# jhbastek/PhysicsInformedDiffusionModels

Hardware: NVIDIA H100
Metric: train samples/s Darcy 64x64 PIDM (higher is better)
Workload: dtype bf16

## Files before the change

include/pidm.h:

```cpp
#ifndef PIDM_H_
#define PIDM_H_

#ifdef __cplusplus
extern "C" {
#endif

#ifndef PIDM_F32
#define PIDM_F32 0
#define PIDM_BF16 1
#endif

const char* pidm_last_error(void);
int pidm_version(void);

int pidm_qsample(const float* x0, const float* noise, const long long* t, const float* sqrt_ab,
                 const float* sqrt_1mab, float* xt, int B, int per_sample, void* stream);
int pidm_posterior_step(const float* x_t, const float* x0_pred, const float* z, float* out, float coef1, float coef2,
                        float sigma, long long n, void* stream);
int pidm_axpby_per_sample(const float* a, const float* x, const float* b, const float* y, const float* c,
                          const float* z, float* out, int B, int per_sample, void* stream);
int pidm_ddim_coefs(const long long* t, const long long* t_next, const float* posterior_mean_coef1,
                    const float* posterior_mean_coef2, const float* sqrt_recip_alphas, const float* noise_mean_coeff,
                    const float* alphas_prod, float* coef_x0, float* coef_x, int B, void* stream);
int pidm_scale(const float* x, const float* alpha_dev, float* out, long long n, void* stream);
// ... 34 lines not shown
                     int transposed, int dtype, void* stream);
int pidm_conv2d_wgrad_simt(const void* x, const void* dy, float* dw, float* dbias, int B, int H, int W, int Cin,
                           int Cin_real, int Ho, int Wo, int Cout, int KH, int KW, int stride, int pad, int transposed,
                           long long w_stride_n, long long w_stride_c, int dtype, void* stream);
int pidm_debug_set_trace(void* buf);
int pidm_conv2d_tc_general(const void* x, const void* w_packed, const float* bias, const void* residual, void* y, int B,
                           int H, int W, int Cin, int Ho, int Wo, int Cout, int KH, int KW, int stride, int pad,
                           int transposed, float* gn_sums, int gn_groups, int gn_sums_zeroed, void* stream);
int pidm_conv2d_tc_general_supported(int B, int H, int W, int Cin, int Ho, int Wo, int Cout, int KH, int KW, int stride,
                                     int pad, int transposed);
int pidm_conv2d_wgrad_tc(const void* a, const void* b, float* dw, int B, int HA, int WA, int CA, int CA_real, int GH,
                         int GW, int CB, int KH, int KW, int a_stride, int pad, long long s_row, long long s_col,
                         void* stream);
int pidm_conv2d_wgrad_tc_supported(int B, int GH, int GW, int CA, int CB, int KH, int KW, int a_stride);
int pidm_colsum(const void* x, float* out, long long M, int C, int dtype, void* stream);

int pidm_groupnorm_silu_fwd(const void* x, const float* gamma, const float* beta, const float* scale_shift,
                            const void* residual, void* y, float* sums, int stats_precomputed, int B, int HW, int C, int G,
                            float eps, int dtype, void* stream);
int pidm_groupnorm_silu_bwd(const void* x, const void* dy, const float* sums, const float* gamma, const float* beta,
                            const float* scale_shift, void* dx, float* dgamma, float* dbeta, float* d_scale_shift,
                            float* dbias_of_producer, float* workspace, int B, int HW, int C, int G, float eps,
                            int dtype, void* stream);
int pidm_layernorm_c_fwd(const void* x, const float* gamma, void* y, long long M, int C, float eps, int dtype, void* stream);
int pidm_layernorm_c_bwd(const void* x, const void* dy, const float* gamma, void* dx, float* dgamma,
                         const void* dx_residual , long long M, int C,
                         float eps, int dtype, void* stream);

int pidm_linattn_fused_supported(int C, int heads, int N, int dtype);
int pidm_linattn_fused_workspace_floats(int B, int N);
int pidm_linattn_fused_fwd(const void* xn, const void* w_qkv, void* out, float* ctx, float* kmax, float* kzinv,
                           float* workspace, int B, int N, void* stream);
int pidm_linattn_fused_bwd(const void* xn, const void* w_qkv, const void* dout, const float* ctx, const float* kmax,
                           const float* kzinv, void* dqkv, float* dctx, int B, int N, void* stream);
int pidm_linattn_workspace_floats(int B, int N, int heads);
int pidm_linattn_fwd(const void* qkv, void* out, float* ctx, float* kmax, float* kzinv, float* workspace, int B, int N,
                     int heads, int dtype, void* stream);
int pidm_linattn_bwd(const void* qkv, const void* dout, const float* ctx, const float* kmax, const float* kzinv,
                     void* dqkv, float* dctx_scratch, int B, int N, int heads, int dtype, void* stream);
int pidm_attn_fwd(const void* qkv, void* out, int B, int n_tokens, int heads, int dtype, void* stream);
int pidm_attn_bwd(const void* qkv, const void* dout, void* dqkv, int B, int n_tokens, int heads, int dtype, void* stream);

int pidm_time_embed_fwd(const long long* t, const float* W1, const float* b1, const float* W2, const float* b2,
                        float* emb, float* h1, float* temb, float* silu_t, int B, int dim, int td, void* stream);
int pidm_time_embed_bwd(const float* d_silu_t, const float* emb, const float* h1, const float* temb, const float* W2,
                        float* dW1, float* db1, float* dW2, float* db2, float* workspace, int B, int dim, int td,
                        int parts, void* stream);
int pidm_mlp_entry_size(void);
int pidm_block_mlps_fwd(const void* table_dev, int n_entries, int max_rows, const float* silu_t, int B, int td,
                        void* stream);
int pidm_block_mlps_bwd(const void* table_dev, int n_entries, int max_rows, const float* silu_t, float* d_silu_t, int B,
                        int td, int parts, void* stream);

int pidm_head_fwd(const void* x, const float* w, const float* bias, float* y, int B, int HW, int C, int O,
                  int sigmoid_last, int dtype, void* stream);
int pidm_head_bwd(const void* x, const float* w, const float* y, const float* dy, void* dx, float* dw, float* db, int B,
                  int HW, int C, int O, int sigmoid_last, int dtype, void* stream);

int pidm_sumsq(const float* x, long long n, float* out, float* workspace, void* stream);
int pidm_adam_ema_step(float* param, float* grad, float* exp_avg, float* exp_avg_sq, float* ema_shadow, long long n,
                       float lr, double beta1, double beta2, float eps, int step, int* step_counter_dev,
                       const float* grad_norm_sq_dev, float grad_scale, float max_norm, float ema_mu,
                       int ema_first_step, int zero_grad, void* stream);

int pidm_mechanics_residual_fwd(const float* u, const float* rho, const float* bcs, const float* KE, float* residual,
                                float* compliance, int B, int nel, void* stream);
int pidm_mechanics_residual_bwd(const float* u, const float* rho, const float* bcs, const float* KE,
// ... 15 lines not shown
```

physicsinformeddiffusionmodels_b200/_lib.py:

```python
import ctypes
import os

import torch

_HERE = os.path.dirname(os.path.abspath(__file__))
LIB_PATH = os.path.join(_HERE, 'libpidm.so')

P = ctypes.c_void_p
I = ctypes.c_int
L = ctypes.c_longlong
F = ctypes.c_float
D = ctypes.c_double

_SIGS = {
    'pidm_qsample': [P, P, P, P, P, P, I, I, P],
    'pidm_posterior_step': [P, P, P, P, F, F, F, L, P],
    'pidm_scale': [P, P, P, L, P],
    'pidm_ddim_coefs': [P, P, P, P, P, P, P, P, P, I, P],
    'pidm_axpby_per_sample': [P, P, P, P, P, P, P, I, I, P],
    'pidm_toy_pidm_loss': [P, P, P, P, P, P, P, P, F, F, F, F, P, P, P, P, P, I, I, P],
    'pidm_fd_stencil': [P, P, I, I, I, F, F, P],
    'pidm_darcy_residual_fwd': [P, P, P, I, I, F, I, I, P],
    'pidm_darcy_residual_bwd': [P, P, P, P, I, I, F, I, I, P],
    'pidm_darcy_jacobian_max': [P, P, I, I, F, I, I, P],
    'pidm_darcy_pidm_loss': [P, P, P, P, P, P, P, F, F, P, P, P, I, I, F, I, I, P],
    'pidm_nchw_to_nhwc': [P, P, I, I, I, I, I, P],
    'pidm_nhwc_to_nchw': [P, P, I, I, I, I, I, P],
    'pidm_add': [P, P, P, L, I, P],
    'pidm_gelu_fwd': [P, P, L, I, P],
    'pidm_gelu_bwd': [P, P, P, L, I, P],
    'pidm_concat_channels': [P, P, P, L, I, I, I, P],
    'pidm_split_channels': [P, P, P, L, I, I, I, P],
    'pidm_pack_entry_size': [],
    'pidm_pack_weights': [P, I, I, P],
    'pidm_pack_pair_entry_size': [],
    'pidm_pack_weights_pairs': [P, P, I, I, I, I, P],
    'pidm_conv2d_simt': [P, P, P, P, P, I, I, I, I, I, I, I, I, I, I, I, I, I, P],
    'pidm_conv2d_wgrad_simt': [P, P, P, P, I, I, I, I, I, I, I, I, I, I, I, I, I, L, L, I, P],
    'pidm_debug_set_trace': [P],
    'pidm_conv2d_tc_general': [P, P, P, P, P, I, I, I, I, I, I, I, I, I, I, I, I, P, I, I, P],
    'pidm_conv2d_tc_general_supported': [I, I, I, I, I, I, I, I, I, I, I, I],
    'pidm_conv2d_wgrad_tc': [P, P, P, I, I, I, I, I, I, I, I, I, I, I, I, L, L, P],
    'pidm_conv2d_wgrad_tc_supported': [I, I, I, I, I, I, I, I],
    'pidm_colsum': [P, P, L, I, I, P],
    'pidm_groupnorm_silu_fwd': [P, P, P, P, P, P, P, I, I, I, I, I, F, I, P],
    'pidm_groupnorm_silu_bwd': [P, P, P, P, P, P, P, P, P, P, P, P, I, I, I, I, F, I, P],
    'pidm_layernorm_c_fwd': [P, P, P, L, I, F, I, P],
    'pidm_layernorm_c_bwd': [P, P, P, P, P, P, L, I, F, I, P],
    'pidm_linattn_workspace_floats': [I, I, I],
    'pidm_linattn_fused_supported': [I, I, I, I],
    'pidm_linattn_fused_workspace_floats': [I, I],
    'pidm_linattn_fused_fwd': [P, P, P, P, P, P, P, I, I, P],
    'pidm_linattn_fused_bwd': [P, P, P, P, P, P, P, P, I, I, P],
    'pidm_linattn_fwd': [P, P, P, P, P, P, I, I, I, I, P],
    'pidm_linattn_bwd': [P, P, P, P, P, P, P, I, I, I, I, P],
    'pidm_attn_fwd': [P, P, I, I, I, I, P],
    'pidm_attn_bwd': [P, P, P, I, I, I, I, P],
    'pidm_time_embed_fwd': [P, P, P, P, P, P, P, P, P, I, I, I, P],
    'pidm_time_embed_bwd': [P, P, P, P, P, P, P, P, P, P, I, I, I, I, P],
    'pidm_mlp_entry_size': [],
    'pidm_block_mlps_fwd': [P, I, I, P, I, I, P],
    'pidm_block_mlps_bwd': [P, I, I, P, P, I, I, I, P],
    'pidm_head_fwd': [P, P, P, P, I, I, I, I, I, I, P],
    'pidm_head_bwd': [P, P, P, P, P, P, P, I, I, I, I, I, I, P],
    'pidm_sumsq': [P, L, P, P, P],
    'pidm_adam_ema_step': [P, P, P, P, P, L, F, D, D, F, I, P, P, F, F, F, I, I, P],
    'pidm_mechanics_residual_fwd': [P, P, P, P, P, P, I, I, P],
    'pidm_mechanics_residual_bwd': [P, P, P, P, P, P, P, P, P, I, I, P],
    'pidm_mech_pidm_loss': [P, P, P, P, P, P, P, P, P, F, F, F, F, P, P, P, P, P, I, I, P],
    'pidm_bilinear_resize_fwd': [P, P, I, I, I, P],
    'pidm_bilinear_resize_bwd': [P, P, I, I, I, P],
    'pidm_version': [],
}
_VALUE_RETURN = {'pidm_pack_entry_size', 'pidm_pack_pair_entry_size', 'pidm_mlp_entry_size', 'pidm_linattn_workspace_floats', 'pidm_version',
                 'pidm_linattn_fused_supported', 'pidm_linattn_fused_workspace_floats',
                 'pidm_conv2d_tc_supported', 'pidm_conv2d_wgrad_tc_supported', 'pidm_conv2d_tc_general_supported'}

if not os.path.exists(LIB_PATH):
    raise ImportError(f'{LIB_PATH} is missing: build it with `python __graft_entry__.py` (nvcc, sm_90a). '
                      'There is no CPU / PyTorch fallback for the PIDM hot path.')

_lib = ctypes.CDLL(LIB_PATH)
_lib.pidm_last_error.restype = ctypes.c_char_p
_lib.pidm_last_error.argtypes = []
for _n, _a in _SIGS.items():
    _f = getattr(_lib, _n)
# ... 39 lines not shown
```

physicsinformeddiffusionmodels_b200/csrc/attention_fused.cu:

```cuda
#define PIDM_PDL_GROUP 1
#include "common.cuh"
#include "mma_util.cuh"
#include "pidm.h"

namespace pidm {

constexpr int LF_C = 32;

__device__ __forceinline__ uint32_t movm_t(uint32_t x) {
    uint32_t y;
    asm volatile("movmatrix.sync.aligned.m8n8.trans.b16 %0, %1;" : "=r"(y) : "r"(x));
    return y;
}

__device__ __forceinline__ void load_w_frags(uint32_t (&w)[2][4][2], const __nv_bfloat16* __restrict__ Wrows, int lane) {
    const int g = lane >> 2, t = lane & 3;
#pragma unroll
    for (int ks = 0; ks < 2; ++ks)
#pragma unroll
        for (int nt = 0; nt < 4; ++nt) {
            const uint32_t* row = reinterpret_cast<const uint32_t*>(Wrows + (size_t)(nt * 8 + g) * LF_C + ks * 16 + 2 * t);
            w[ks][nt][0] = __ldg(row);
            w[ks][nt][1] = __ldg(row + 4);
        }
// ... 300 lines not shown
        __syncwarp();
        issue(it + LFO_STAGES);
        float cq[2][4][4];
        project<2>(cq, ax, wq);
#pragma unroll
        for (int mt = 0; mt < 2; ++mt) {
            frag_softmax(cq[mt], scale);
            uint32_t a[2][4];
            c_to_a(a, cq[mt]);
            float c[4][4];
#pragma unroll
            for (int i = 0; i < 4; ++i)
#pragma unroll
                for (int k = 0; k < 4; ++k) c[i][k] = 0.f;
#pragma unroll
            for (int ks = 0; ks < 2; ++ks)
#pragma unroll
                for (int nt = 0; nt < 4; ++nt) mma_bf16(c[nt], a[ks], bf[ks][nt][0], bf[ks][nt][1]);
#pragma unroll
            for (int nt = 0; nt < 4; ++nt) {
                __nv_bfloat16* o = Os + (size_t)(mt * 16 + g) * LW_PITCH + nt * 8 + 2 * t;
                *reinterpret_cast<uint32_t*>(o) = pack_bf16(c[nt][0], c[nt][1]);
                *reinterpret_cast<uint32_t*>(o + 8 * LW_PITCH) = pack_bf16(c[nt][2], c[nt][3]);
            }
        }
        __syncwarp();
        lw_store<32>(odst + (size_t)it * 32 * LM_HID, LM_HID, Os, lane);
        __syncwarp();
    }
}

constexpr int LFB_ROWS = 16;
constexpr int LFB_STAGES = 4;
constexpr int LFB_STAGE_ELEMS = 2 * LFB_ROWS * LW_PITCH;
constexpr int LFB_OUT_ELEMS = 3 * LFB_ROWS * LW_PITCH;
__global__ void __launch_bounds__(256) laf_bwd_kernel(const __nv_bfloat16* __restrict__ xn, const __nv_bfloat16* __restrict__ W,
                                                      const __nv_bfloat16* __restrict__ dout, const float* __restrict__ ctx,
                                                      const float* __restrict__ dctx, const float* __restrict__ kmax,
                                                      const float* __restrict__ kzinv, __nv_bfloat16* __restrict__ dqkv,
                                                      int N, int chunk_px, float scale) {
    pdl_trigger();
    pdl_wait();
    extern __shared__ __align__(16) unsigned char raw[];
    const int b = blockIdx.y, chunk = blockIdx.x, lane = threadIdx.x & 31, h = threadIdx.x >> 5;
    __nv_bfloat16* ring = reinterpret_cast<__nv_bfloat16*>(raw) + (size_t)h * (LFB_STAGES * LFB_STAGE_ELEMS + LFB_OUT_ELEMS);
    __nv_bfloat16* Os = ring + LFB_STAGES * LFB_STAGE_ELEMS;
    float* scd = reinterpret_cast<float*>(raw + (size_t)LM_HEADS * (LFB_STAGES * LFB_STAGE_ELEMS + LFB_OUT_ELEMS) * 2) + h * LM_D;
    const int n_begin = chunk * chunk_px, n_end = min(N, n_begin + chunk_px);
    const int n_tiles = (n_end - n_begin) / LFB_ROWS;
    const size_t pix0 = (size_t)b * N + n_begin;
    const __nv_bfloat16* xsrc = xn + pix0 * LF_C;
    const __nv_bfloat16* gsrc = dout + pix0 * LM_HID + h * LM_D;
    __nv_bfloat16* ddst = dqkv + pix0 * 3 * LM_HID + h * LM_D;
    auto issue = [&](int it) {
        if (it < n_tiles) {
            __nv_bfloat16* buf = ring + (size_t)(it % LFB_STAGES) * LFB_STAGE_ELEMS;
            lw_issue<LFB_ROWS>(buf, xsrc + (size_t)it * LFB_ROWS * LF_C, LF_C, lane);
            lw_issue<LFB_ROWS>(buf + LFB_ROWS * LW_PITCH, gsrc + (size_t)it * LFB_ROWS * LM_HID, LM_HID, lane);
        }
        cp_commit();
    };
#pragma unroll
    for (int s = 0; s < LFB_STAGES; ++s) issue(s);
    const float* cg = ctx + ((size_t)b * LM_HEADS + h) * LM_D * LM_D;
    const float* dg = dctx + ((size_t)b * LM_HEADS + h) * LM_D * LM_D;
    {
        float s = 0.f;
#pragma unroll
        for (int e = 0; e < LM_D; e += 4) {
            const float4 x = *reinterpret_cast<const float4*>(dg + lane * LM_D + e);
            const float4 y = *reinterpret_cast<const float4*>(cg + lane * LM_D + e);
            s += x.x * y.x + x.y * y.y + x.z * y.z + x.w * y.w;
        }
        scd[lane] = s;
    }
    __syncwarp();
    float Mc[8], Zc[8], cdc[8];
    load_cols(Mc, kmax + (size_t)b * LM_HID + h * LM_D, lane);
    load_cols(Zc, kzinv + (size_t)b * LM_HID + h * LM_D, lane);
    load_cols(cdc, scd, lane);
    uint32_t wq[2][4][2], wk[2][4][2], wv[2][4][2];
    load_w_frags(wq, W + (size_t)(h * LM_D) * LF_C, lane);
    load_w_frags(wk, W + (size_t)(LM_HID + h * LM_D) * LF_C, lane);
    load_w_frags(wv, W + (size_t)(2 * LM_HID + h * LM_D) * LF_C, lane);
    uint32_t bc[2][4][2], bd[2][4][2], bt[2][4][2];
#pragma unroll
    for (int ks = 0; ks < 2; ++ks)
#pragma unroll
        for (int nt = 0; nt < 4; ++nt) {
            frag_b_global<false>(bc[ks][nt], cg, ks * 16, nt * 8, lane);
            frag_b_global<false>(bd[ks][nt], dg, ks * 16, nt * 8, lane);
            frag_b_global<true>(bt[ks][nt], dg, ks * 16, nt * 8, lane);
        }
    const int g = lane >> 2, t = lane & 3;
    const float invN = 1.f / (float)N;
    __nv_bfloat16* Oq = Os;
    __nv_bfloat16* Ok = Os + LFB_ROWS * LW_PITCH;
    __nv_bfloat16* Ov = Os + 2 * LFB_ROWS * LW_PITCH;
    for (int it = 0; it < n_tiles; ++it) {
        cp_wait<LFB_STAGES - 1>();
        __syncwarp();
        const __nv_bfloat16* buf = ring + (size_t)(it % LFB_STAGES) * LFB_STAGE_ELEMS;
        uint32_t ax[1][2][4], ag[2][4];
        load_x_frags<1>(ax, buf, lane);
        frag_a_rowmajor(ag[0], buf + LFB_ROWS * LW_PITCH, LW_PITCH, 0, 0, lane);
        frag_a_rowmajor(ag[1], buf + LFB_ROWS * LW_PITCH, LW_PITCH, 0, 16, lane);
        __syncwarp();
        issue(it + LFB_STAGES);
        float c1[1][4][4], c2[4][4];
        project<1>(c1, ax, wq);
        frag_softmax(c1[0], 1.f);
#pragma unroll
        for (int nt = 0; nt < 4; ++nt) {
#pragma unroll
            for (int i = 0; i < 4; ++i) c2[nt][i] = 0.f;
#pragma unroll
            for (int ks = 0; ks < 2; ++ks) mma_bf16(c2[nt], ag[ks], bc[ks][nt][0], bc[ks][nt][1]);
        }
#pragma unroll
        for (int half = 0; half < 2; ++half) {
            float dot = 0.f;
#pragma unroll
            for (int nt = 0; nt < 4; ++nt)
                dot += c1[0][nt][half * 2] * c2[nt][half * 2] + c1[0][nt][half * 2 + 1] * c2[nt][half * 2 + 1];
            dot += __shfl_xor_sync(0xffffffffu, dot, 1);
            dot += __shfl_xor_sync(0xffffffffu, dot, 2);
#pragma unroll
            for (int nt = 0; nt < 4; ++nt)
                *reinterpret_cast<uint32_t*>(Oq + (g + half * 8) * LW_PITCH + nt * 8 + 2 * t) =
                    pack_bf16(scale * c1[0][nt][half * 2] * (c2[nt][half * 2] - dot),
                              scale * c1[0][nt][half * 2 + 1] * (c2[nt][half * 2 + 1] - dot));
        }
        uint32_t av[2][4], ak[2][4];
        project<1>(c1, ax, wv);
        c_to_a(av, c1[0]);
#pragma unroll
        for (int nt = 0; nt < 4; ++nt) {
#pragma unroll
            for (int i = 0; i < 4; ++i) c2[nt][i] = 0.f;
#pragma unroll
            for (int ks = 0; ks < 2; ++ks) mma_bf16(c2[nt], av[ks], bd[ks][nt][0], bd[ks][nt][1]);
        }
        project<1>(c1, ax, wk);
#pragma unroll
        for (int nt = 0; nt < 4; ++nt)
#pragma unroll
            for (int i = 0; i < 4; ++i)
                c1[0][nt][i] = __expf(c1[0][nt][i] - Mc[nt * 2 + (i & 1)]) * Zc[nt * 2 + (i & 1)];
        c_to_a(ak, c1[0]);
#pragma unroll
        for (int half = 0; half < 2; ++half)
#pragma unroll
            for (int nt = 0; nt < 4; ++nt)
                *reinterpret_cast<uint32_t*>(Ok + (g + half * 8) * LW_PITCH + nt * 8 + 2 * t) =
                    pack_bf16(c1[0][nt][half * 2] * (c2[nt][half * 2] * invN - cdc[nt * 2]),
                              c1[0][nt][half * 2 + 1] * (c2[nt][half * 2 + 1] * invN - cdc[nt * 2 + 1]));
#pragma unroll
        for (int nt = 0; nt < 4; ++nt) {
#pragma unroll
            for (int i = 0; i < 4; ++i) c2[nt][i] = 0.f;
#pragma unroll
            for (int ks = 0; ks < 2; ++ks) mma_bf16(c2[nt], ak[ks], bt[ks][nt][0], bt[ks][nt][1]);
        }
#pragma unroll
        for (int half = 0; half < 2; ++half)
#pragma unroll
            for (int nt = 0; nt < 4; ++nt)
                *reinterpret_cast<uint32_t*>(Ov + (g + half * 8) * LW_PITCH + nt * 8 + 2 * t) =
                    pack_bf16(c2[nt][half * 2] * invN, c2[nt][half * 2 + 1] * invN);
        __syncwarp();
        __nv_bfloat16* d = ddst + (size_t)it * LFB_ROWS * 3 * LM_HID;
        lw_store<LFB_ROWS>(d, 3 * LM_HID, Oq, lane);
        lw_store<LFB_ROWS>(d + LM_HID, 3 * LM_HID, Ok, lane);
        lw_store<LFB_ROWS>(d + 2 * LM_HID, 3 * LM_HID, Ov, lane);
        __syncwarp();
    }
}

constexpr size_t LAF_STATS_SMEM = (size_t)LM_HEADS * LFS_STAGES * LW_TILE * 2;
constexpr size_t LAF_OUT_SMEM = (size_t)LM_HEADS * (LFO_STAGES + 1) * LW_TILE * 2;
constexpr size_t LAF_BWD_SMEM = (size_t)LM_HEADS * (LFB_STAGES * LFB_STAGE_ELEMS + LFB_OUT_ELEMS) * 2 + (size_t)LM_HEADS * LM_D * 4;

static int laf_attrs() {
    static bool done = false;
    if (!done) {
        PIDM_CUDA(cudaFuncSetAttribute(laf_kmax_kernel, cudaFuncAttributeMaxDynamicSharedMemorySize, (int)LAF_STATS_SMEM));
        PIDM_CUDA(cudaFuncSetAttribute(laf_ctx_kernel<0>, cudaFuncAttributeMaxDynamicSharedMemorySize, (int)LfcCfg<0>::SMEM));
        PIDM_CUDA(cudaFuncSetAttribute(laf_ctx_kernel<1>, cudaFuncAttributeMaxDynamicSharedMemorySize, (int)LfcCfg<1>::SMEM));
        PIDM_CUDA(cudaFuncSetAttribute(laf_out_kernel, cudaFuncAttributeMaxDynamicSharedMemorySize, (int)LAF_OUT_SMEM));
        PIDM_CUDA(cudaFuncSetAttribute(laf_bwd_kernel, cudaFuncAttributeMaxDynamicSharedMemorySize, (int)LAF_BWD_SMEM));
        done = true;
    }
    return 0;
}

static int laf_chunk_px(int B, int N, int ctas_per_sm) {
    int k = (num_sms() * ctas_per_sm) / B;
    if (k < 1) k = 1;
    int px = ((N + k - 1) / k + 31) / 32 * 32;
    if (px < 64) px = 64;
    if (px > N) px = N;
    return px;
}
static int laf_stat_chunks(int N) {
    int c = N / 128;
    if (c < 1) c = 1;
    if (c > 16) c = 16;
    return c;
}

}
using namespace pidm;

extern "C" int pidm_linattn_fused_supported(int C, int heads, int N, int dtype) {
    return (C == LF_C && heads == LM_HEADS && dtype == PIDM_BF16 && N % 128 == 0) ? 1 : 0;
}

extern "C" int pidm_linattn_fused_workspace_floats(int B, int N) { return B * laf_stat_chunks(N) * LM_HID; }

extern "C" int pidm_linattn_fused_fwd(const void* xn, const void* w_qkv, void* out, float* ctx, float* kmax, float* kzinv,
                                      float* workspace, int B, int N, void* stream) {
    PIDM_REQUIRE(N % 128 == 0, "linattn_fused: N must be a multiple of 128 (got %d)", N);
    cudaStream_t st = (cudaStream_t)stream;
    if (int e = laf_attrs()) return e;
    const float scale = 0.17677669529663687f;
    const __nv_bfloat16* x = (const __nv_bfloat16*)xn;
    const __nv_bfloat16* w = (const __nv_bfloat16*)w_qkv;
    PIDM_CUDA(cudaMemsetAsync(ctx, 0, (size_t)B * LM_HEADS * LM_D * LM_D * sizeof(float), st));
    PIDM_CUDA(cudaMemsetAsync(kzinv, 0, (size_t)B * LM_HID * sizeof(float), st));
    const int chunks = laf_stat_chunks(N);
    const int rpc = N / chunks;
    PIDM_REQUIRE(rpc % 32 == 0 && rpc * chunks == N, "linattn_fused: bad statistics chunking for N=%d", N);
    PIDM_CUDA(launch_pdl(laf_kmax_kernel, dim3(dim3(chunks, B)), dim3(256), (size_t)(LAF_STATS_SMEM), st, x, w, workspace, N, rpc));
    const int cpx = laf_chunk_px(B, N, 2);
    PIDM_CUDA(launch_pdl(laf_ctx_kernel<0>, dim3(dim3((N + cpx - 1) / cpx, B)), dim3(256), (size_t)(LfcCfg<0>::SMEM), st, x, w, nullptr, workspace, chunks, kmax, kzinv,
                                                                             ctx, N, cpx, scale));
    PIDM_CUDA(launch_pdl(laf_finalize_kernel, dim3((B * LM_HID + 7) / 8), dim3(256), (size_t)(0), st, ctx, kzinv, B * LM_HID));
    const int opx = laf_chunk_px(B, N, 3);
    PIDM_CUDA(launch_pdl(laf_out_kernel, dim3(dim3((N + opx - 1) / opx, B)), dim3(256), (size_t)(LAF_OUT_SMEM), st, x, w, ctx, (__nv_bfloat16*)out, N, opx, scale));
    PIDM_LAUNCH_CHECK("linattn_fused_fwd");
    return 0;
}

extern "C" int pidm_linattn_fused_bwd(const void* xn, const void* w_qkv, const void* dout, const float* ctx,
                                      const float* kmax, const float* kzinv, void* dqkv, float* dctx, int B, int N,
                                      void* stream) {
    PIDM_REQUIRE(N % 128 == 0, "linattn_fused: N must be a multiple of 128 (got %d)", N);
    cudaStream_t st = (cudaStream_t)stream;
    if (int e = laf_attrs()) return e;
    const float scale = 0.17677669529663687f;
    const __nv_bfloat16* x = (const __nv_bfloat16*)xn;
    const __nv_bfloat16* w = (const __nv_bfloat16*)w_qkv;
    PIDM_CUDA(cudaMemsetAsync(dctx, 0, (size_t)B * LM_HEADS * LM_D * LM_D * sizeof(float), st));
    const int cpx = laf_chunk_px(B, N, 2);
    PIDM_CUDA(launch_pdl(laf_ctx_kernel<1>, dim3(dim3((N + cpx - 1) / cpx, B)), dim3(256), (size_t)(LfcCfg<1>::SMEM), st, x, w, (const __nv_bfloat16*)dout, nullptr, 0,
                                                                             nullptr, nullptr, dctx, N, cpx, scale));
    const int bpx = laf_chunk_px(B, N, 1);
    PIDM_CUDA(launch_pdl(laf_bwd_kernel, dim3(dim3((N + bpx - 1) / bpx, B)), dim3(256), (size_t)(LAF_BWD_SMEM), st, x, w, (const __nv_bfloat16*)dout, ctx, dctx, kmax,
                                                                          kzinv, (__nv_bfloat16*)dqkv, N, bpx, scale));
    PIDM_LAUNCH_CHECK("linattn_fused_bwd");
    return 0;
}
```

physicsinformeddiffusionmodels_b200/ops.py:

```python
import os

import torch

from . import _lib
from ._lib import call, stream

_TC_HARD_OFF = os.environ.get('PIDM_DISABLE_TC') == '1'
_STATE = {'act_dtype': torch.bfloat16, 'use_tc': not _TC_HARD_OFF}


def set_precision(name):
    _STATE['act_dtype'] = {'bf16': torch.bfloat16, 'fp32': torch.float32}[name]


def set_tensor_core_conv(flag):
    _STATE['use_tc'] = bool(flag) and not _TC_HARD_OFF


def act_dtype():
    return _STATE['act_dtype']


def _code(t):
    return _lib.DTYPE_CODE[t.dtype]
# ... 370 lines not shown
        return out

    @staticmethod
    def backward(ctx, dout):
        qkv, ctxm, kmax, kzinv = ctx.saved_tensors
        B, H, W, _ = qkv.shape
        dout = dout.contiguous()
        dqkv = torch.empty_like(qkv)
        dctx = torch.empty_like(ctxm)
        call('pidm_linattn_bwd', qkv, dout, ctxm, kmax, kzinv, dqkv, dctx, B, H * W, ctx.heads, _code(qkv), stream())
        return dqkv, None


class _LinAttnFused(torch.autograd.Function):

    @staticmethod
    def forward(ctx, xn, weight, spec, heads):
        B, H, W, C = xn.shape
        N = H * W
        out = torch.empty(B, H, W, heads * 32, device=xn.device, dtype=xn.dtype)
        ctxm = torch.empty(B, heads, 32, 32, device=xn.device, dtype=torch.float32)
        kmax = torch.empty(B, heads, 32, device=xn.device, dtype=torch.float32)
        kzinv = torch.empty_like(kmax)
        ws = torch.empty(call('pidm_linattn_fused_workspace_floats', B, N), device=xn.device, dtype=torch.float32)
        call('pidm_linattn_fused_fwd', xn, spec.wp_fwd, out, ctxm, kmax, kzinv, ws, B, N, stream())
        ctx.save_for_backward(xn, weight, ctxm, kmax, kzinv)
        ctx.spec, ctx.heads = spec, heads
        return out

    @staticmethod
    def backward(ctx, dout):
        xn, weight, ctxm, kmax, kzinv = ctx.saved_tensors
        spec = ctx.spec
        B, H, W, C = xn.shape
        dout = dout.contiguous()
        dqkv = torch.empty(B, H, W, 3 * ctx.heads * 32, device=xn.device, dtype=xn.dtype)
        dctx = torch.empty_like(ctxm)
        call('pidm_linattn_fused_bwd', xn, spec.wp_fwd, dout, ctxm, kmax, kzinv, dqkv, dctx, B, H * W, stream())
        g = (B, H, W, C, H, W, spec.cout, 1, 1, 1, 0)
        dx, gw_ret, _ = _conv_backward(xn, weight, None, spec, g, dqkv, ctx.needs_input_grad[0])
        return dx, gw_ret, None, None


def linear_attention_fused_supported(xn, spec, heads):
    B, H, W, C = xn.shape
    return (_STATE['use_tc'] and xn.is_cuda and spec.kh == 1 and spec.kw == 1 and spec.cout == 3 * heads * 32
            and bool(call('pidm_linattn_fused_supported', C, heads, H * W, _code(xn))))


def linear_attention_fused(xn, weight, spec, heads):
    return _LinAttnFused.apply(xn.contiguous(), weight, spec, heads)


def linear_attention(qkv, heads):
    return _LinAttn.apply(qkv.contiguous(), heads)


class _Attn(torch.autograd.Function):
    @staticmethod
    def forward(ctx, qkv, heads):
        B, H, W, C3 = qkv.shape
        out = torch.empty(B, H, W, heads * 32, device=qkv.device, dtype=qkv.dtype)
        call('pidm_attn_fwd', qkv, out, B, H * W, heads, _code(qkv), stream())
        ctx.save_for_backward(qkv)
        ctx.heads = heads
        return out

    @staticmethod
    def backward(ctx, dout):
        (qkv,) = ctx.saved_tensors
        B, H, W, _ = qkv.shape
        dqkv = torch.empty_like(qkv)
        call('pidm_attn_bwd', qkv, dout.contiguous(), dqkv, B, H * W, ctx.heads, _code(qkv), stream())
        return dqkv, None
# ... 187 lines not shown
```

Measured before the change: 6230.

## Fuse qkv conv backward into linear-attention backward and add recomputing wgrad kernels

The fused linear-attention backward no longer writes dqkv to global memory and runs a separate 1x1 conv backward. It now multiplies dq/dk/dv by the shared-memory weights in registers to produce dxn directly, with a cross-warp reduction through shared memory. Weight gradients come from two new kernels that recompute dq/dk/dv from xn and dout and atomically accumulate x^T·g into the grad buffer, launched on a separate wgrad stream. This removes the dqkv round trip and the extra conv launches, but the recompute duplicates projection and softmax work and adds atomics and block-wide syncs.

```diff
diff --git a/include/pidm.h b/include/pidm.h
--- a/include/pidm.h
+++ b/include/pidm.h
@@ -90,7 +90,10 @@
 int pidm_linattn_fused_fwd(const void* xn, const void* w_qkv, void* out, float* ctx, float* kmax, float* kzinv,
                            float* workspace, int B, int N, void* stream);
 int pidm_linattn_fused_bwd(const void* xn, const void* w_qkv, const void* dout, const float* ctx, const float* kmax,
-                           const float* kzinv, void* dqkv, float* dctx, int B, int N, void* stream);
+                           const float* kzinv, void* dxn, float* dctx, int B, int N, void* stream);
+int pidm_linattn_fused_wgrad(const void* xn, const void* w_qkv, const void* dout, const float* ctx, const float* dctx,
+                             const float* kmax, const float* kzinv, float* grad_w, int B, int N, long long w_stride_n,
+                             long long w_stride_c, void* stream);
 int pidm_linattn_workspace_floats(int B, int N, int heads);
 int pidm_linattn_fwd(const void* qkv, void* out, float* ctx, float* kmax, float* kzinv, float* workspace, int B, int N,
                      int heads, int dtype, void* stream);
diff --git a/physicsinformeddiffusionmodels_b200/_lib.py b/physicsinformeddiffusionmodels_b200/_lib.py
--- a/physicsinformeddiffusionmodels_b200/_lib.py
+++ b/physicsinformeddiffusionmodels_b200/_lib.py
@@ -52,6 +52,7 @@
     'pidm_linattn_fused_workspace_floats': [I, I],
     'pidm_linattn_fused_fwd': [P, P, P, P, P, P, P, I, I, P],
     'pidm_linattn_fused_bwd': [P, P, P, P, P, P, P, P, I, I, P],
+    'pidm_linattn_fused_wgrad': [P, P, P, P, P, P, P, P, I, I, L, L, P],
     'pidm_linattn_fwd': [P, P, P, P, P, P, I, I, I, I, P],
     'pidm_linattn_bwd': [P, P, P, P, P, P, P, I, I, I, I, P],
     'pidm_attn_fwd': [P, P, I, I, I, I, P],
diff --git a/physicsinformeddiffusionmodels_b200/csrc/attention_fused.cu b/physicsinformeddiffusionmodels_b200/csrc/attention_fused.cu
--- a/physicsinformeddiffusionmodels_b200/csrc/attention_fused.cu
+++ b/physicsinformeddiffusionmodels_b200/csrc/attention_fused.cu
@@ -356,53 +356,140 @@
 
 constexpr int LFB_ROWS = 16;
 constexpr int LFB_STAGES = 4;
-constexpr int LFB_STAGE_ELEMS = 2 * LFB_ROWS * LW_PITCH;
-constexpr int LFB_OUT_ELEMS = 3 * LFB_ROWS * LW_PITCH;
+constexpr int LFB_TILE = LFB_ROWS * LW_PITCH;
+
+struct LfbTile {
+    uint32_t ax[1][2][4], ag[2][4];
+};
+__device__ __forceinline__ void lfb_dq(float (&dq)[4][4], const LfbTile& tl, const uint32_t (&wq)[2][4][2],
+                                       const uint32_t (&bc)[2][4][2], float scale) {
+    float c1[1][4][4], c2[4][4];
+    project<1>(c1, tl.ax, wq);
+    frag_softmax(c1[0], 1.f);
+#pragma unroll
+    for (int nt = 0; nt < 4; ++nt) {
+#pragma unroll
+        for (int i = 0; i < 4; ++i) c2[nt][i] = 0.f;
+#pragma unroll
+        for (int ks = 0; ks < 2; ++ks) mma_bf16(c2[nt], tl.ag[ks], bc[ks][nt][0], bc[ks][nt][1]);
+    }
+#pragma unroll
+    for (int half = 0; half < 2; ++half) {
+        float dot = 0.f;
+#pragma unroll
+        for (int nt = 0; nt < 4; ++nt)
+            dot += c1[0][nt][half * 2] * c2[nt][half * 2] + c1[0][nt][half * 2 + 1] * c2[nt][half * 2 + 1];
+        dot += __shfl_xor_sync(0xffffffffu, dot, 1);
+        dot += __shfl_xor_sync(0xffffffffu, dot, 2);
+#pragma unroll
+        for (int nt = 0; nt < 4; ++nt)
+#pragma unroll
+            for (int j = 0; j < 2; ++j) dq[nt][half * 2 + j] = scale * c1[0][nt][half * 2 + j] * (c2[nt][half * 2 + j] - dot);
+    }
+}
+__device__ __forceinline__ void lfb_dkdv(float (&dk)[4][4], float (&dv)[4][4], const uint32_t (&ax)[1][2][4],
+                                         const uint32_t (&wk)[2][4][2], const uint32_t (&wv)[2][4][2],
+                                         const uint32_t (&bd)[2][4][2], const uint32_t (&bt)[2][4][2],
+                                         const float (&Mc)[8], const float (&Zc)[8], const float (&cdc)[8], float invN) {
+    float c1[1][4][4];
+    uint32_t a[2][4];
+    project<1>(c1, ax, wv);
+    c_to_a(a, c1[0]);
+#pragma unroll
+    for (int nt = 0; nt < 4; ++nt) {
+#pragma unroll
+        for (int i = 0; i < 4; ++i) dk[nt][i] = 0.f;
+#pragma unroll
+        for (int ks = 0; ks < 2; ++ks) mma_bf16(dk[nt], a[ks], bd[ks][nt][0], bd[ks][nt][1]);
+    }
+    project<1>(c1, ax, wk);
+#pragma unroll
+    for (int nt = 0; nt < 4; ++nt)
+#pragma unroll
+        for (int i = 0; i < 4; ++i) {
+            c1[0][nt][i] = __expf(c1[0][nt][i] - Mc[nt * 2 + (i & 1)]) * Zc[nt * 2 + (i & 1)];
+            dk[nt][i] = c1[0][nt][i] * (dk[nt][i] * invN - cdc[nt * 2 + (i & 1)]);
+        }
+    c_to_a(a, c1[0]);
+#pragma unroll
+    for (int nt = 0; nt < 4; ++nt) {
+#pragma unroll
+        for (int i = 0; i < 4; ++i) dv[nt][i] = 0.f;
+#pragma unroll
+        for (int ks = 0; ks < 2; ++ks) mma_bf16(dv[nt], a[ks], bt[ks][nt][0], bt[ks][nt][1]);
+#pragma unroll
+        for (int i = 0; i < 4; ++i) dv[nt][i] *= invN;
+    }
+}
+__device__ __forceinline__ void lfb_cd(float (&cdc)[8], float* scd, const float* __restrict__ cg, const float* __restrict__ dg,
+                                       int lane) {
+    float s = 0.f;
+#pragma unroll
+    for (int e = 0; e < LM_D; e += 4) {
+        const float4 x = *reinterpret_cast<const float4*>(dg + lane * LM_D + e);
+        const float4 y = *reinterpret_cast<const float4*>(cg + lane * LM_D + e);
+        s += x.x * y.x + x.y * y.y + x.z * y.z + x.w * y.w;
+    }
+    scd[lane] = s;
+    __syncwarp();
+    load_cols(cdc, scd, lane);
+}
+
+constexpr int LFB_STAGE_ELEMS = (1 + LM_HEADS) * LFB_TILE;
+constexpr int LFB_W_PITCH = LF_C + 8;
+constexpr int LFB_R_PITCH = LF_C + 8;
+constexpr size_t LAF_BWD_SMEM = (size_t)LFB_STAGES * LFB_STAGE_ELEMS * 2 + (size_t)3 * LM_HID * LFB_W_PITCH * 2 +
+                                (size_t)LM_HEADS * LFB_ROWS * LFB_R_PITCH * 4 + (size_t)LM_HEADS * LM_D * 4;
+
+__device__ __forceinline__ void mma_w(float (&c)[4][4], const uint32_t (&g)[2][4], const __nv_bfloat16* Wh, int lane) {
+#pragma unroll
+    for (int kd = 0; kd < 2; ++kd)
+#pragma unroll
+        for (int np = 0; np < 2; ++np) {
+            uint32_t bw[4];
+            frag_b_krows(bw, Wh, LFB_W_PITCH, kd * 16, np * 16, lane);
+            mma_bf16(c[2 * np], g[kd], bw[0], bw[1]);
+            mma_bf16(c[2 * np + 1], g[kd], bw[2], bw[3]);
+        }
+}
+
 __global__ void __launch_bounds__(256) laf_bwd_kernel(const __nv_bfloat16* __restrict__ xn, const __nv_bfloat16* __restrict__ W,
                                                       const __nv_bfloat16* __restrict__ dout, const float* __restrict__ ctx,
                                                       const float* __restrict__ dctx, const float* __restrict__ kmax,
-                                                      const float* __restrict__ kzinv, __nv_bfloat16* __restrict__ dqkv,
+                                                      const float* __restrict__ kzinv, __nv_bfloat16* __restrict__ dxn,
                                                       int N, int chunk_px, float scale) {
     pdl_trigger();
     pdl_wait();
     extern __shared__ __align__(16) unsigned char raw[];
     const int b = blockIdx.y, chunk = blockIdx.x, lane = threadIdx.x & 31, h = threadIdx.x >> 5;
-    __nv_bfloat16* ring = reinterpret_cast<__nv_bfloat16*>(raw) + (size_t)h * (LFB_STAGES * LFB_STAGE_ELEMS + LFB_OUT_ELEMS);
-    __nv_bfloat16* Os = ring + LFB_STAGES * LFB_STAGE_ELEMS;
-    float* scd = reinterpret_cast<float*>(raw + (size_t)LM_HEADS * (LFB_STAGES * LFB_STAGE_ELEMS + LFB_OUT_ELEMS) * 2) + h * LM_D;
+    __nv_bfloat16* ring = reinterpret_cast<__nv_bfloat16*>(raw);
+    __nv_bfloat16* Ws = ring + LFB_STAGES * LFB_STAGE_ELEMS;
+    float* R = reinterpret_cast<float*>(Ws + 3 * LM_HID * LFB_W_PITCH);
+    float* scd = R + LM_HEADS * LFB_ROWS * LFB_R_PITCH + h * LM_D;
     const int n_begin = chunk * chunk_px, n_end = min(N, n_begin + chunk_px);
     const int n_tiles = (n_end - n_begin) / LFB_ROWS;
     const size_t pix0 = (size_t)b * N + n_begin;
     const __nv_bfloat16* xsrc = xn + pix0 * LF_C;
     const __nv_bfloat16* gsrc = dout + pix0 * LM_HID + h * LM_D;
-    __nv_bfloat16* ddst = dqkv + pix0 * 3 * LM_HID + h * LM_D;
+    for (int i = threadIdx.x; i < 3 * LM_HID * (LF_C / 8); i += blockDim.x)
+        cp_async16(Ws + (i >> 2) * LFB_W_PITCH + (i & 3) * 8, W + (size_t)(i >> 2) * LF_C + (i & 3) * 8);
+    cp_commit();
     auto issue = [&](int it) {
         if (it < n_tiles) {
             __nv_bfloat16* buf = ring + (size_t)(it % LFB_STAGES) * LFB_STAGE_ELEMS;
-            lw_issue<LFB_ROWS>(buf, xsrc + (size_t)it * LFB_ROWS * LF_C, LF_C, lane);
-            lw_issue<LFB_ROWS>(buf + LFB_ROWS * LW_PITCH, gsrc + (size_t)it * LFB_ROWS * LM_HID, LM_HID, lane);
+            if (h == 0) lw_issue<LFB_ROWS>(buf, xsrc + (size_t)it * LFB_ROWS * LF_C, LF_C, lane);
+            lw_issue<LFB_ROWS>(buf + (1 + h) * LFB_TILE, gsrc + (size_t)it * LFB_ROWS * LM_HID, LM_HID, lane);
         }
         cp_commit();
     };
 #pragma unroll
-    for (int s = 0; s < LFB_STAGES; ++s) issue(s);
+    for (int s = 0; s < LFB_STAGES - 1; ++s) issue(s);
     const float* cg = ctx + ((size_t)b * LM_HEADS + h) * LM_D * LM_D;
     const float* dg = dctx + ((size_t)b * LM_HEADS + h) * LM_D * LM_D;
-    {
-        float s = 0.f;
-#pragma unroll
-        for (int e = 0; e < LM_D; e += 4) {
-            const float4 x = *reinterpret_cast<const float4*>(dg + lane * LM_D + e);
-            const float4 y = *reinterpret_cast<const float4*>(cg + lane * LM_D + e);
-            s += x.x * y.x + x.y * y.y + x.z * y.z + x.w * y.w;
-        }
-        scd[lane] = s;
-    }
-    __syncwarp();
     float Mc[8], Zc[8], cdc[8];
+    lfb_cd(cdc, scd, cg, dg, lane);
     load_cols(Mc, kmax + (size_t)b * LM_HID + h * LM_D, lane);
     load_cols(Zc, kzinv + (size_t)b * LM_HID + h * LM_D, lane);
-    load_cols(cdc, scd, lane);
     uint32_t wq[2][4][2], wk[2][4][2], wv[2][4][2];
     load_w_frags(wq, W + (size_t)(h * LM_D) * LF_C, lane);
     load_w_frags(wk, W + (size_t)(LM_HID + h * LM_D) * LF_C, lane);
@@ -418,92 +505,190 @@
         }
     const int g = lane >> 2, t = lane & 3;
     const float invN = 1.f / (float)N;
-    __nv_bfloat16* Oq = Os;
-    __nv_bfloat16* Ok = Os + LFB_ROWS * LW_PITCH;
-    __nv_bfloat16* Ov = Os + 2 * LFB_ROWS * LW_PITCH;
+    const __nv_bfloat16* Wq = Ws + (size_t)(h * LM_D) * LFB_W_PITCH;
+    const __nv_bfloat16* Wk = Wq + (size_t)LM_HID * LFB_W_PITCH;
+    const __nv_bfloat16* Wv = Wk + (size_t)LM_HID * LFB_W_PITCH;
+    float* Rw = R + h * LFB_ROWS * LFB_R_PITCH;
+    const int rrow = threadIdx.x >> 4, rcol = (threadIdx.x & 15) * 2;
+    for (int it = 0; it < n_tiles; ++it) {
+        cp_wait<LFB_STAGES - 2>();
+        __syncthreads();
+        issue(it + LFB_STAGES - 1);
+        const __nv_bfloat16* buf = ring + (size_t)(it % LFB_STAGES) * LFB_STAGE_ELEMS;
+        LfbTile tl;
+        load_x_frags<1>(tl.ax, buf, lane);
+        frag_a_rowmajor(tl.ag[0], buf + (1 + h) * LFB_TILE, LW_PITCH, 0, 0, lane);
+        frag_a_rowmajor(tl.ag[1], buf + (1 + h) * LFB_TILE, LW_PITCH, 0, 16, lane);
+        float dx[4][4];
+#pragma unroll
+        for (int nt = 0; nt < 4; ++nt)
+#pragma unroll
+            for (int i = 0; i < 4; ++i) dx[nt][i] = 0.f;
+        uint32_t a[2][4];
+        {
+            float dq[4][4];
+            lfb_dq(dq, tl, wq, bc, scale);
+            c_to_a(a, dq);
+            mma_w(dx, a, Wq, lane);
+        }
+        {
+            float dk[4][4], dv[4][4];
+            lfb_dkdv(dk, dv, tl.ax, wk, wv, bd, bt, Mc, Zc, cdc, invN);
+            c_to_a(a, dk);
+            mma_w(dx, a, Wk, lane);
+            c_to_a(a, dv);
+            mma_w(dx, a, Wv, lane);
+        }
+#pragma unroll
+        for (int nt = 0; nt < 4; ++nt)
+#pragma unroll
+            for (int half = 0; half < 2; ++half)
+                *reinterpret_cast<float2*>(Rw + (g + half * 8) * LFB_R_PITCH + nt * 8 + 2 * t) =
+                    make_float2(dx[nt][half * 2], dx[nt][half * 2 + 1]);
+        __syncthreads();
+        float sx = 0.f, sy = 0.f;
+#pragma unroll
+        for (int w = 0; w < LM_HEADS; ++w) {
+            const float2 v = *reinterpret_cast<const float2*>(R + (w * LFB_ROWS + rrow) * LFB_R_PITCH + rcol);
+            sx += v.x;
+            sy += v.y;
+        }
+        *reinterpret_cast<uint32_t*>(dxn + (pix0 + (size_t)it * LFB_ROWS + rrow) * LF_C + rcol) = pack_bf16(sx, sy);
+    }
+}
+
+template <int PART>
+struct LfwCfg {
+    static constexpr int MATS = PART == 0 ? 1 : 2;
+    static constexpr int STAGE_ELEMS = (PART == 0 ? 2 : 1) * LFB_TILE;
+    static constexpr int S_PITCH = LM_D + 1;
+    static_assert(LFB_STAGES * STAGE_ELEMS * 2 >= LM_D * S_PITCH * 4, "the epilogue staging reuses the tile ring");
+    static constexpr size_t SMEM = (size_t)LM_HEADS * (LFB_STAGES * STAGE_ELEMS * 2 + LM_D * 4);
+};
+
+__device__ __forceinline__ void acc_gtx(float (&acc)[2][4][4], const float (&gf)[4][4], const uint32_t (&bx)[2][4]) {
+#pragma unroll
+    for (int md = 0; md < 2; ++md) {
+        uint32_t a[4];
+        a[0] = movm_t(pack_bf16(gf[2 * md][0], gf[2 * md][1]));
+        a[1] = movm_t(pack_bf16(gf[2 * md + 1][0], gf[2 * md + 1][1]));
+        a[2] = movm_t(pack_bf16(gf[2 * md][2], gf[2 * md][3]));
+        a[3] = movm_t(pack_bf16(gf[2 * md + 1][2], gf[2 * md + 1][3]));
+#pragma unroll
+        for (int np = 0; np < 2; ++np) {
+            mma_bf16(acc[md][2 * np], a, bx[np][0], bx[np][1]);
+            mma_bf16(acc[md][2 * np + 1], a, bx[np][2], bx[np][3]);
+        }
+    }
+}
+
+template <int PART>
+__global__ void __launch_bounds__(256) laf_wgrad_kernel(const __nv_bfloat16* __restrict__ xn, const __nv_bfloat16* __restrict__ W,
+                                                        const __nv_bfloat16* __restrict__ dout, const float* __restrict__ ctx,
+                                                        const float* __restrict__ dctx, const float* __restrict__ kmax,
+                                                        const float* __restrict__ kzinv, float* __restrict__ grad_w, int N,
+                                                        int chunk_px, long long w_stride_n, long long w_stride_c, float scale) {
+    pdl_trigger();
+    pdl_wait();
+    extern __shared__ __align__(16) unsigned char raw[];
+    constexpr int MATS = LfwCfg<PART>::MATS, STAGE_ELEMS = LfwCfg<PART>::STAGE_ELEMS, S_PITCH = LfwCfg<PART>::S_PITCH;
+    const int b = blockIdx.y, chunk = blockIdx.x, lane = threadIdx.x & 31, h = threadIdx.x >> 5;
+    __nv_bfloat16* ring = reinterpret_cast<__nv_bfloat16*>(raw) + (size_t)h * (LFB_STAGES * STAGE_ELEMS);
+    float* scd = reinterpret_cast<float*>(raw + (size_t)LM_HEADS * LFB_STAGES * STAGE_ELEMS * 2) + h * LM_D;
+    const int n_begin = chunk * chunk_px, n_end = min(N, n_begin + chunk_px);
+    const int n_tiles = (n_end - n_begin) / LFB_ROWS;
+    const size_t pix0 = (size_t)b * N + n_begin;
+    const __nv_bfloat16* xsrc = xn + pix0 * LF_C;
+    const __nv_bfloat16* gsrc = dout + pix0 * LM_HID + h * LM_D;
+    auto issue = [&](int it) {
+        if (it < n_tiles) {
+            __nv_bfloat16* buf = ring + (size_t)(it % LFB_STAGES) * STAGE_ELEMS;
+            lw_issue<LFB_ROWS>(buf, xsrc + (size_t)it * LFB_ROWS * LF_C, LF_C, lane);
+            if (PART == 0) lw_issue<LFB_ROWS>(buf + LFB_TILE, gsrc + (size_t)it * LFB_ROWS * LM_HID, LM_HID, lane);
+        }
+        cp_commit();
+    };
+#pragma unroll
+    for (int s = 0; s < LFB_STAGES; ++s) issue(s);
+    const float* cg = ctx + ((size_t)b * LM_HEADS + h) * LM_D * LM_D;
+    const float* dg = dctx + ((size_t)b * LM_HEADS + h) * LM_D * LM_D;
+    float Mc[8], Zc[8], cdc[8];
+    uint32_t w0[2][4][2], w1[2][4][2];
+    uint32_t b0[2][4][2], b1[2][4][2];
+    if (PART == 0) {
+        load_w_frags(w0, W + (size_t)(h * LM_D) * LF_C, lane);
+    } else {
+        lfb_cd(cdc, scd, cg, dg, lane);
+        load_cols(Mc, kmax + (size_t)b * LM_HID + h * LM_D, lane);
+        load_cols(Zc, kzinv + (size_t)b * LM_HID + h * LM_D, lane);
+        load_w_frags(w0, W + (size_t)(LM_HID + h * LM_D) * LF_C, lane);
+        load_w_frags(w1, W + (size_t)(2 * LM_HID + h * LM_D) * LF_C, lane);
+    }
+#pragma unroll
+    for (int ks = 0; ks < 2; ++ks)
+#pragma unroll
+        for (int nt = 0; nt < 4; ++nt) {
+            frag_b_global<false>(b0[ks][nt], PART == 0 ? cg : dg, ks * 16, nt * 8, lane);
+            if (PART == 1) frag_b_global<true>(b1[ks][nt], dg, ks * 16, nt * 8, lane);
+        }
+    const float invN = 1.f / (float)N;
+    float acc[MATS][2][4][4];
+#pragma unroll
+    for (int m = 0; m < MATS; ++m)
+#pragma unroll
+        for (int i = 0; i < 2; ++i)
+#pragma unroll
+            for (int j = 0; j < 4; ++j)
+#pragma unroll
+                for (int k = 0; k < 4; ++k) acc[m][i][j][k] = 0.f;
     for (int it = 0; it < n_tiles; ++it) {
         cp_wait<LFB_STAGES - 1>();
         __syncwarp();
-        const __nv_bfloat16* buf = ring + (size_t)(it % LFB_STAGES) * LFB_STAGE_ELEMS;
-        uint32_t ax[1][2][4], ag[2][4];
-        load_x_frags<1>(ax, buf, lane);
-        frag_a_rowmajor(ag[0], buf + LFB_ROWS * LW_PITCH, LW_PITCH, 0, 0, lane);
-        frag_a_rowmajor(ag[1], buf + LFB_ROWS * LW_PITCH, LW_PITCH, 0, 16, lane);
+        const __nv_bfloat16* buf = ring + (size_t)(it % LFB_STAGES) * STAGE_ELEMS;
+        LfbTile tl;
+        load_x_frags<1>(tl.ax, buf, lane);
+        uint32_t bx[2][4];
+        frag_b_krows(bx[0], buf, LW_PITCH, 0, 0, lane);
+        frag_b_krows(bx[1], buf, LW_PITCH, 0, 16, lane);
+        if (PART == 0) {
+            frag_a_rowmajor(tl.ag[0], buf + LFB_TILE, LW_PITCH, 0, 0, lane);
+            frag_a_rowmajor(tl.ag[1], buf + LFB_TILE, LW_PITCH, 0, 16, lane);
+        }
         __syncwarp();
         issue(it + LFB_STAGES);
-        float c1[1][4][4], c2[4][4];
-        project<1>(c1, ax, wq);
-        frag_softmax(c1[0], 1.f);
-#pragma unroll
-        for (int nt = 0; nt < 4; ++nt) {
-#pragma unroll
-            for (int i = 0; i < 4; ++i) c2[nt][i] = 0.f;
-#pragma unroll
-            for (int ks = 0; ks < 2; ++ks) mma_bf16(c2[nt], ag[ks], bc[ks][nt][0], bc[ks][nt][1]);
-        }
-#pragma unroll
-        for (int half = 0; half < 2; ++half) {
-            float dot = 0.f;
-#pragma unroll
-            for (int nt = 0; nt < 4; ++nt)
-                dot += c1[0][nt][half * 2] * c2[nt][half * 2] + c1[0][nt][half * 2 + 1] * c2[nt][half * 2 + 1];
-            dot += __shfl_xor_sync(0xffffffffu, dot, 1);
-            dot += __shfl_xor_sync(0xffffffffu, dot, 2);
-#pragma unroll
-            for (int nt = 0; nt < 4; ++nt)
-                *reinterpret_cast<uint32_t*>(Oq + (g + half * 8) * LW_PITCH + nt * 8 + 2 * t) =
-                    pack_bf16(scale * c1[0][nt][half * 2] * (c2[nt][half * 2] - dot),
-                              scale * c1[0][nt][half * 2 + 1] * (c2[nt][half * 2 + 1] - dot));
-        }
-        uint32_t av[2][4], ak[2][4];
-        project<1>(c1, ax, wv);
-        c_to_a(av, c1[0]);
-#pragma unroll
-        for (int nt = 0; nt < 4; ++nt) {
-#pragma unroll
-            for (int i = 0; i < 4; ++i) c2[nt][i] = 0.f;
-#pragma unroll
-            for (int ks = 0; ks < 2; ++ks) mma_bf16(c2[nt], av[ks], bd[ks][nt][0], bd[ks][nt][1]);
-        }
-        project<1>(c1, ax, wk);
-#pragma unroll
-        for (int nt = 0; nt < 4; ++nt)
-#pragma unroll
-            for (int i = 0; i < 4; ++i)
-                c1[0][nt][i] = __expf(c1[0][nt][i] - Mc[nt * 2 + (i & 1)]) * Zc[nt * 2 + (i & 1)];
-        c_to_a(ak, c1[0]);
-#pragma unroll
-        for (int half = 0; half < 2; ++half)
-#pragma unroll
-            for (int nt = 0; nt < 4; ++nt)
-                *reinterpret_cast<uint32_t*>(Ok + (g + half * 8) * LW_PITCH + nt * 8 + 2 * t) =
-                    pack_bf16(c1[0][nt][half * 2] * (c2[nt][half * 2] * invN - cdc[nt * 2]),
-                              c1[0][nt][half * 2 + 1] * (c2[nt][half * 2 + 1] * invN - cdc[nt * 2 + 1]));
-#pragma unroll
-        for (int nt = 0; nt < 4; ++nt) {
-#pragma unroll
-            for (int i = 0; i < 4; ++i) c2[nt][i] = 0.f;
-#pragma unroll
-            for (int ks = 0; ks < 2; ++ks) mma_bf16(c2[nt], ak[ks], bt[ks][nt][0], bt[ks][nt][1]);
-        }
-#pragma unroll
-        for (int half = 0; half < 2; ++half)
-#pragma unroll
-            for (int nt = 0; nt < 4; ++nt)
-                *reinterpret_cast<uint32_t*>(Ov + (g + half * 8) * LW_PITCH + nt * 8 + 2 * t) =
-                    pack_bf16(c2[nt][half * 2] * invN, c2[nt][half * 2 + 1] * invN);
-        __syncwarp();
-        __nv_bfloat16* d = ddst + (size_t)it * LFB_ROWS * 3 * LM_HID;
-        lw_store<LFB_ROWS>(d, 3 * LM_HID, Oq, lane);
-        lw_store<LFB_ROWS>(d + LM_HID, 3 * LM_HID, Ok, lane);
-        lw_store<LFB_ROWS>(d + 2 * LM_HID, 3 * LM_HID, Ov, lane);
+        if (PART == 0) {
+            float dq[4][4];
+            lfb_dq(dq, tl, w0, b0, scale);
+            acc_gtx(acc[0], dq, bx);
+        } else {
+            float dk[4][4], dv[4][4];
+            lfb_dkdv(dk, dv, tl.ax, w0, w1, b0, b1, Mc, Zc, cdc, invN);
+            acc_gtx(acc[0], dk, bx);
+            acc_gtx(acc[MATS - 1], dv, bx);
+        }
+    }
+    cp_wait<0>();
+    __syncwarp();
+    float* S = reinterpret_cast<float*>(ring);
+    const int g = lane >> 2, t = lane & 3;
+#pragma unroll
+    for (int m = 0; m < MATS; ++m) {
+#pragma unroll
+        for (int md = 0; md < 2; ++md)
+#pragma unroll
+            for (int nc = 0; nc < 4; ++nc)
+#pragma unroll
+                for (int i = 0; i < 4; ++i) S[(md * 16 + g + 8 * (i >> 1)) * S_PITCH + nc * 8 + 2 * t + (i & 1)] = acc[m][md][nc][i];
+        __syncwarp();
+        float* dst = grad_w + (long long)((PART + m) * LM_HID + h * LM_D) * w_stride_n + lane * w_stride_c;
+#pragma unroll 4
+        for (int d = 0; d < LM_D; ++d) atomicAdd(dst + d * w_stride_n, S[d * S_PITCH + lane]);
         __syncwarp();
     }
 }
 
 constexpr size_t LAF_STATS_SMEM = (size_t)LM_HEADS * LFS_STAGES * LW_TILE * 2;
 constexpr size_t LAF_OUT_SMEM = (size_t)LM_HEADS * (LFO_STAGES + 1) * LW_TILE * 2;
-constexpr size_t LAF_BWD_SMEM = (size_t)LM_HEADS * (LFB_STAGES * LFB_STAGE_ELEMS + LFB_OUT_ELEMS) * 2 + (size_t)LM_HEADS * LM_D * 4;
 
 static int laf_attrs() {
     static bool done = false;
@@ -513,6 +698,8 @@
         PIDM_CUDA(cudaFuncSetAttribute(laf_ctx_kernel<1>, cudaFuncAttributeMaxDynamicSharedMemorySize, (int)LfcCfg<1>::SMEM));
         PIDM_CUDA(cudaFuncSetAttribute(laf_out_kernel, cudaFuncAttributeMaxDynamicSharedMemorySize, (int)LAF_OUT_SMEM));
         PIDM_CUDA(cudaFuncSetAttribute(laf_bwd_kernel, cudaFuncAttributeMaxDynamicSharedMemorySize, (int)LAF_BWD_SMEM));
+        PIDM_CUDA(cudaFuncSetAttribute(laf_wgrad_kernel<0>, cudaFuncAttributeMaxDynamicSharedMemorySize, (int)LfwCfg<0>::SMEM));
+        PIDM_CUDA(cudaFuncSetAttribute(laf_wgrad_kernel<1>, cudaFuncAttributeMaxDynamicSharedMemorySize, (int)LfwCfg<1>::SMEM));
         done = true;
     }
     return 0;
@@ -567,7 +754,7 @@
 }
 
 extern "C" int pidm_linattn_fused_bwd(const void* xn, const void* w_qkv, const void* dout, const float* ctx,
-                                      const float* kmax, const float* kzinv, void* dqkv, float* dctx, int B, int N,
+                                      const float* kmax, const float* kzinv, void* dxn, float* dctx, int B, int N,
                                       void* stream) {
     PIDM_REQUIRE(N % 128 == 0, "linattn_fused: N must be a multiple of 128 (got %d)", N);
     cudaStream_t st = (cudaStream_t)stream;
@@ -581,7 +768,27 @@
                                                                              nullptr, nullptr, dctx, N, cpx, scale));
     const int bpx = laf_chunk_px(B, N, 1);
     PIDM_CUDA(launch_pdl(laf_bwd_kernel, dim3(dim3((N + bpx - 1) / bpx, B)), dim3(256), (size_t)(LAF_BWD_SMEM), st, x, w, (const __nv_bfloat16*)dout, ctx, dctx, kmax,
-                                                                          kzinv, (__nv_bfloat16*)dqkv, N, bpx, scale));
+                                                                          kzinv, (__nv_bfloat16*)dxn, N, bpx, scale));
     PIDM_LAUNCH_CHECK("linattn_fused_bwd");
     return 0;
 }
+
+extern "C" int pidm_linattn_fused_wgrad(const void* xn, const void* w_qkv, const void* dout, const float* ctx,
+                                        const float* dctx, const float* kmax, const float* kzinv, float* grad_w, int B,
+                                        int N, long long w_stride_n, long long w_stride_c, void* stream) {
+    PIDM_REQUIRE(N % 128 == 0, "linattn_fused: N must be a multiple of 128 (got %d)", N);
+    cudaStream_t st = (cudaStream_t)stream;
+    if (int e = laf_attrs()) return e;
+    const float scale = 0.17677669529663687f;
+    const __nv_bfloat16* x = (const __nv_bfloat16*)xn;
+    const __nv_bfloat16* w = (const __nv_bfloat16*)w_qkv;
+    const __nv_bfloat16* g = (const __nv_bfloat16*)dout;
+    const int px = laf_chunk_px(B, N, 1);
+    const dim3 grid((N + px - 1) / px, B);
+    PIDM_CUDA(launch_pdl(laf_wgrad_kernel<0>, grid, dim3(256), LfwCfg<0>::SMEM, st, x, w, g, ctx, dctx, kmax, kzinv, grad_w, N,
+                         px, w_stride_n, w_stride_c, scale));
+    PIDM_CUDA(launch_pdl(laf_wgrad_kernel<1>, grid, dim3(256), LfwCfg<1>::SMEM, st, x, w, g, ctx, dctx, kmax, kzinv, grad_w, N,
+                         px, w_stride_n, w_stride_c, scale));
+    PIDM_LAUNCH_CHECK("linattn_fused_wgrad");
+    return 0;
+}
diff --git a/physicsinformeddiffusionmodels_b200/ops.py b/physicsinformeddiffusionmodels_b200/ops.py
--- a/physicsinformeddiffusionmodels_b200/ops.py
+++ b/physicsinformeddiffusionmodels_b200/ops.py
@@ -426,14 +426,16 @@
     def backward(ctx, dout):
         xn, weight, ctxm, kmax, kzinv = ctx.saved_tensors
         spec = ctx.spec
-        B, H, W, C = xn.shape
+        B, H, W, _ = xn.shape
         dout = dout.contiguous()
-        dqkv = torch.empty(B, H, W, 3 * ctx.heads * 32, device=xn.device, dtype=xn.dtype)
+        dx = torch.empty_like(xn)
         dctx = torch.empty_like(ctxm)
-        call('pidm_linattn_fused_bwd', xn, spec.wp_fwd, dout, ctxm, kmax, kzinv, dqkv, dctx, B, H * W, stream())
-        g = (B, H, W, C, H, W, spec.cout, 1, 1, 1, 0)
-        dx, gw_ret, _ = _conv_backward(xn, weight, None, spec, g, dqkv, ctx.needs_input_grad[0])
-        return dx, gw_ret, None, None
+        call('pidm_linattn_fused_bwd', xn, spec.wp_fwd, dout, ctxm, kmax, kzinv, dx, dctx, B, H * W, stream())
+        gw_buf, gw_ret = _grad_buffer(weight)
+        ws = _wgrad_stream(xn, spec.wp_fwd, dout, ctxm, dctx, kmax, kzinv)
+        call('pidm_linattn_fused_wgrad', xn, spec.wp_fwd, dout, ctxm, dctx, kmax, kzinv, gw_buf, B, H * W,
+             spec.w_stride_n, spec.w_stride_c, ws)
+        return (dx if ctx.needs_input_grad[0] else None), gw_ret, None, None
 
 
 def linear_attention_fused_supported(xn, spec, heads):
```

Result: faster. 6525, median of 6 (+4.7%).
